# mhnazeri/PMoE

Measured on AMD Instinct MI355X. Metric: samples/sec fwd+bwd, 256x256 RGB 4-expert PMoE, higher is better.
Workload: dtype bf16; 1 GPU; 4-expert MoE (PMoE experts), 256x256x3 x4 frames, batch 64/GPU, fwd+moe_loss+bwd, dropout 0.3; global_batch=64, parallelism=dp1

## Files before the change

### include/pmoe_hip.h

```cpp
#ifndef PMOE_HIP_H
#define PMOE_HIP_H
#include <stdint.h>
#ifdef __cplusplus
extern "C" {
#endif

#define PMOE_DT_BF16 0
#define PMOE_DT_F32 1

#define PMOE_ERR_ARG (-1)
#define PMOE_ERR_UNSUPPORTED (-2)

#define PMOE_ACT_NONE 0
#define PMOE_ACT_RELU 1
#define PMOE_ACT_ELU 2
#define PMOE_ACT_TANH 3
#define PMOE_ACT_SIGMOID 4

#define PMOE_RES_NONE 0
#define PMOE_RES_ADD 1
#define PMOE_RES_DRELU 2
#define PMOE_RES_DELU 3
#define PMOE_RES_DTANH 4
#define PMOE_RES_DSIGMOID 5
// ... 4 lines not shown
int pmoe_version(void);
const char* pmoe_error_string(int code);
int pmoe_abi_sizeof(int which);

typedef struct pmoe_conv_desc {
    const void* in;
    const void* w;
    void* out;
    const void* res;
    const float* bias;
    float* stats;
    int32_t n, h, w_, cin;
    int32_t ho, wo, cout, coutp;
    int32_t in_ld, in_coff, out_ld, out_coff, res_ld, res_coff;
    int32_t ipe;
    int32_t in_shared;
    int32_t ks, stride, pad, dilate;
    int32_t act, res_mode;
    float drop_p;
    uint64_t seed;
    int32_t dtype;
    int32_t w_fp8;
    float in_scale;
    const float* out_scale;
    int32_t in_fp8;
    const float* bn_coef;
    int32_t bn_ipe;
    int32_t shuffle_c;
} pmoe_conv_desc;

int pmoe_conv2d_igemm(const pmoe_conv_desc* d, void* stream);
int pmoe_conv2d_stat_rows(const pmoe_conv_desc* d);
int pmoe_conv2d_plan(const pmoe_conv_desc* d);

typedef struct pmoe_wgrad_desc {
    const void* x;
    const void* dy;
    float* dw_ws;
    int32_t n, h, w_, cin, cinp;
    int32_t ho, wo, cout, coutp;
    int32_t x_ld, x_coff, dy_ld, dy_coff;
    int32_t ipe, x_shared;
    int32_t ks, stride, pad;
    int32_t dtype;
    int32_t per_image;
    float* part_ws;
    int64_t part_ws_floats;
    float* grads;
    int32_t cout_real, cin_real;
    int32_t defer_fold;
    int32_t bn_fused;
    const void* bn_z;
    const float* bn_coef;
    const float* bn_c1;
    const float* bn_c2;
    int32_t bn_z_ld;
} pmoe_wgrad_desc;
int pmoe_conv2d_wgrad(const pmoe_wgrad_desc* d, void* stream);
int pmoe_conv2d_wgrad_fold(const pmoe_wgrad_desc* d, void* stream);
int64_t pmoe_conv2d_wgrad_ws_floats(const pmoe_wgrad_desc* d);
int pmoe_conv2d_wgrad_plan(const pmoe_wgrad_desc* d);

int pmoe_mlp_wgrad(const void* x, const void* dy, float* grads, float* bias_grads, int32_t n, int32_t ipe, int32_t x_shared,
                   int32_t cin, int32_t cout, int32_t cin_real, int32_t cout_real, int32_t x_ld, int32_t x_coff,
                   int32_t dy_ld, int32_t dy_coff, int32_t dtype, void* stream);

// ... 241 lines not shown
```

### pmoe_amd/csrc/api.hip

```cpp
#include "common.h"
#include "kernels.h"

static ConvArgs to_args(const pmoe_conv_desc* d) {
    ConvArgs a;
    a.in = d->in; a.w = d->w; a.out = d->out; a.res = d->res; a.bias = d->bias; a.stats = d->stats;
    a.N = d->n; a.H = d->h; a.W = d->w_; a.Cin = d->cin;
    a.Ho = d->ho; a.Wo = d->wo; a.Cout = d->cout; a.CoutP = d->coutp;
    a.in_ld = d->in_ld; a.in_coff = d->in_coff; a.out_ld = d->out_ld; a.out_coff = d->out_coff;
    a.res_ld = d->res_ld; a.res_coff = d->res_coff;
    a.ipe = d->ipe; a.in_shared = d->in_shared;
    a.ks = d->ks; a.stride = d->stride; a.pad = d->pad; a.dilate = d->dilate;
    a.act = d->act; a.res_mode = (d->res || d->res_mode == PMOE_RES_INBN) ? d->res_mode : PMOE_RES_NONE;
    a.drop_p = d->drop_p; a.seed = d->seed;
    a.oscale = d->out_scale; a.in_scale = d->in_scale; a.w_fp8 = d->w_fp8; a.in_fp8 = d->in_fp8;
    a.bn = d->bn_coef; a.bn_ipe = d->bn_ipe > 0 ? d->bn_ipe : d->ipe;
    a.lTW = a.lTH = a.TN = a.n_groups = a.tiles_y = a.tiles_x = 0;
    a.kh = a.kw = d->ks; a.use_tapmap = 0; a.tapmap[0] = a.tapmap[1] = a.tapmap[2] = a.tapmap[3] = 0;
    a.out_step = 1; a.out_offy = a.out_offx = 0; a.OH = d->ho; a.OW = d->wo; a.prefetch = 0; a.stagger = 0;
    a.shuf_c = d->shuffle_c > 0 ? d->shuffle_c : 0;
    return a;
}

static int check_conv(const pmoe_conv_desc* d) {
    if (!d || !d->in || !d->w || !d->out) return PMOE_ERR_ARG;
    if (d->n <= 0 || d->h <= 0 || d->w_ <= 0 || d->ho <= 0 || d->wo <= 0 || d->ipe <= 0) return PMOE_ERR_ARG;
    const int ve = d->dtype == PMOE_DT_BF16 ? 8 : 4;
    if (d->in_fp8 && (!d->w_fp8 || d->dtype != PMOE_DT_BF16 || d->in_ld % 16 || d->in_coff % 16)) return PMOE_ERR_ARG;
    if (d->in_ld % ve || d->in_coff % ve || d->out_ld % ve || d->out_coff % ve) return PMOE_ERR_ARG;
    if (d->res && (d->res_ld % ve || d->res_coff % ve)) return PMOE_ERR_ARG;
    if (d->shuffle_c > 0 ? (d->cout != 4 * d->shuffle_c || d->shuffle_c % ve || d->out_coff + d->shuffle_c > d->out_ld || d->cout > d->coutp)
                         : (d->cout > d->coutp || d->out_coff + d->cout > d->out_ld)) return PMOE_ERR_ARG;
    if (d->in_coff + d->cin > d->in_ld) return PMOE_ERR_ARG;
    if (d->drop_p < 0.f || d->drop_p >= 1.f) return PMOE_ERR_ARG;
    if (d->res && d->res_mode == PMOE_RES_DBN &&
        (!d->bn_coef || !d->stats || d->dtype != PMOE_DT_BF16 || (d->bn_ipe > 0 && (d->bn_ipe % d->ipe || d->n % d->bn_ipe))))
        return PMOE_ERR_ARG;
    if (d->res_mode == PMOE_RES_INBN &&
        (d->res || !d->bn_coef || d->dtype != PMOE_DT_BF16 || (d->bias && d->ks != 1) || d->act != PMOE_ACT_NONE || d->drop_p != 0.f || d->in_shared ||
         d->w_fp8 || d->dilate || (d->bn_ipe > 0 && (d->bn_ipe % d->ipe || d->n % d->bn_ipe))))
        return PMOE_ERR_ARG;
    if (!d->dilate) {
        if (d->ho != (d->h + 2 * d->pad - d->ks) / d->stride + 1) return PMOE_ERR_ARG;
        if (d->wo != (d->w_ + 2 * d->pad - d->ks) / d->stride + 1) return PMOE_ERR_ARG;
    }
    return 0;
}

extern "C" {

int pmoe_version(void) { return PMOE_ABI_VERSION; }

int pmoe_abi_sizeof(int which) {
// ... 3 lines not shown
}

const char* pmoe_error_string(int code) {
    if (code == 0) return "ok";
    if (code == PMOE_ERR_ARG) return "pmoe: invalid argument (shape / alignment / pointer)";
    if (code == PMOE_ERR_UNSUPPORTED) return "pmoe: unsupported configuration (no tile fits LDS)";
    if (code > 0) return hipGetErrorString((hipError_t)code);
    return "pmoe: unknown error";
}

int pmoe_conv2d_igemm(const pmoe_conv_desc* d, void* stream) {
    int rc = check_conv(d);
    if (rc) return rc;
    return conv_igemm_launch(to_args(d), d->dtype, (hipStream_t)stream);
}

static ConvArgs to_plan_args(const pmoe_conv_desc* d) {
    ConvArgs a = to_args(d);
    if (a.in_ld <= 0) a.in_ld = a.in_coff + a.Cin;
    if (a.out_ld <= 0) a.out_ld = a.out_coff + a.Cout;
    return a;
}

int pmoe_conv2d_stat_rows(const pmoe_conv_desc* d) {
    if (!d || d->ipe <= 0) return PMOE_ERR_ARG;
    return conv_igemm_mblocks(to_plan_args(d), d->dtype);
}

int pmoe_conv2d_plan(const pmoe_conv_desc* d) {
    if (!d || d->ipe <= 0) return PMOE_ERR_ARG;
    return conv_igemm_plan(to_plan_args(d), d->dtype);
}

static int to_wgrad_args(const pmoe_wgrad_desc* d, WgradArgs& a) {
    if (!d || d->ipe <= 0) return PMOE_ERR_ARG;
    const int ve = d->dtype == PMOE_DT_BF16 ? 8 : 4;
    if (d->x_ld % ve || d->x_coff % ve || d->dy_ld % ve || d->dy_coff % ve) return PMOE_ERR_ARG;
    if (d->x_coff + d->cin > d->x_ld || d->dy_coff + d->cout > d->dy_ld) return PMOE_ERR_ARG;
    if (d->ho != (d->h + 2 * d->pad - d->ks) / d->stride + 1) return PMOE_ERR_ARG;
    if (d->wo != (d->w_ + 2 * d->pad - d->ks) / d->stride + 1) return PMOE_ERR_ARG;
    a.x = d->x; a.dy = d->dy; a.dw = d->dw_ws; a.part = d->part_ws; a.part_floats = d->part_ws_floats;
    a.N = d->n; a.H = d->h; a.W = d->w_; a.Cin = d->cin; a.CinP = d->cinp;
    a.Ho = d->ho; a.Wo = d->wo; a.Cout = d->cout; a.CoutP = d->coutp;
    a.x_ld = d->x_ld; a.x_coff = d->x_coff; a.dy_ld = d->dy_ld; a.dy_coff = d->dy_coff;
    a.ipe = d->ipe; a.x_shared = d->x_shared;
    a.ks = d->ks; a.stride = d->stride; a.pad = d->pad; a.per_image = d->per_image;
    a.grads = d->grads; a.cout_real = d->cout_real; a.cin_real = d->cin_real; a.defer_fold = d->defer_fold;
    if (a.grads && (a.per_image || a.cout_real <= 0 || a.cin_real <= 0 || a.cout_real > a.CoutP || a.cin_real > a.CinP)) return PMOE_ERR_ARG;
    a.lTW = a.lTH = a.TN = a.n_groups = a.tiles_y = a.tiles_x = a.mb_per_wg = 0;
    a.slice_fastest = 0;
    return 0;
}

static WgradBn to_wgrad_bn(const pmoe_wgrad_desc* d) { return {d->bn_fused, d->bn_z_ld, d->bn_z, d->bn_coef, d->bn_c1, d->bn_c2}; }

int pmoe_conv2d_wgrad(const pmoe_wgrad_desc* d, void* stream) {
    WgradArgs a;
    const int rc = to_wgrad_args(d, a);
    if (rc) return rc;
    if (!d->x || !d->dy || !d->dw_ws) return PMOE_ERR_ARG;
    return conv_wgrad_launch(a, d->dtype, to_wgrad_bn(d), (hipStream_t)stream);
}

int pmoe_conv2d_wgrad_fold(const pmoe_wgrad_desc* d, void* stream) {
    WgradArgs a;
    const int rc = to_wgrad_args(d, a);
// ... 19 lines not shown
```

### pmoe_amd/csrc/conv_igemm.hip

```cpp
#include "conv_common.h"
#include <stdlib.h>
#include <string.h>
#include "kernels.h"

template <int LOG_RB> __device__ __forceinline__ int swz(int x) { return swz_chunk<LOG_RB, 0>(x); }

template <typename T> struct Mma;
template <> struct Mma<bf16> {
    static __device__ __forceinline__ void run(const v4i& a, const v4i& b, f32x16& c) {
        c = __builtin_amdgcn_mfma_f32_32x32x16_bf16(__builtin_bit_cast(bf16x8, a), __builtin_bit_cast(bf16x8, b), c, 0, 0, 0);
    }
};
template <> struct Mma<float> {
    static __device__ __forceinline__ void run(const v4i& a, const v4i& b, f32x16& c) {
        const f32x4 fa = __builtin_bit_cast(f32x4, a), fb = __builtin_bit_cast(f32x4, b);
#pragma unroll
        for (int j = 0; j < 4; ++j) c = __builtin_amdgcn_mfma_f32_32x32x2f32(fa[j], fb[j], c, 0, 0, 0);
    }
};

template <> struct Mma<fp8> {
    static __device__ __forceinline__ void run(const v4i& a, const v4i& b, f32x16& c) {
        typedef long l2 __attribute__((ext_vector_type(2)));
        const l2 la = __builtin_bit_cast(l2, a), lb = __builtin_bit_cast(l2, b);
        c = __builtin_amdgcn_mfma_f32_32x32x16_fp8_fp8(la[0], lb[0], c, 0, 0, 0);
        c = __builtin_amdgcn_mfma_f32_32x32x16_fp8_fp8(la[1], lb[1], c, 0, 0, 0);
    }
};

#ifdef PMOE_STAMP
#define STAMP_INIT unsigned long long st_prev = __builtin_amdgcn_s_memtime(); unsigned st_acc[5] = {0, 0, 0, 0, 0};
#define LAP(i) { const unsigned long long st_t = __builtin_amdgcn_s_memtime(); st_acc[i] += (unsigned)(st_t - st_prev); st_prev = st_t; }
#else
#define STAMP_INIT
#define LAP(i)
// ... 315 lines not shown
        for (int i = 0; i < VE; ++i) {
#pragma unroll
            for (int off = CPO; off < 64; off <<= 1) {
                s1[i] += __shfl_xor(s1[i], off);
                s2[i] += __shfl_xor(s2[i], off);
            }
        }
        if (CPO >= 64 || lane < CPO) {
#pragma unroll
            for (int i = 0; i < VE; ++i) {
                red[(wave * 2 + 0) * BN + cc * VE + i] = s1[i];
                red[(wave * 2 + 1) * BN + cc * VE + i] = s2[i];
            }
        }
        __syncthreads();
        if (tid < 2 * BN) {
            const int which = tid / BN, c = tid % BN;
            float s = 0.f;
#pragma unroll
            for (int w = 0; w < WM * WN; ++w) s += red[(w * 2 + which) * BN + c];
            if (cout0 + c < a.CoutP) a.stats[((size_t)mb * 2 + which) * a.CoutP + cout0 + c] = s;
        }
    }
}

template <typename T, int LOG_RB, int WM, int WN, typename TL = T>
__global__ void __launch_bounds__(WM * WN * 64) conv_igemm_kernel(const ConvArgs a) {
    conv_igemm_body<T, LOG_RB, WM, WN, false, TL>(a);
}

template <typename T, int LOG_RB, typename TL = T>
__global__ void __launch_bounds__(512, 4) conv_igemm_lite_kernel(const ConvArgs a) {
    conv_igemm_body<T, LOG_RB, 4, 2, true, TL>(a);
}

template <typename T, int LOG_RB, typename TL = T>
static int launch_lite(const ConvArgs& a, int mblocks, size_t smem, hipStream_t st) {
    auto k = conv_igemm_lite_kernel<T, LOG_RB, TL>;
    HIP_RET((ensure_dyn_lds<conv_igemm_lite_kernel<T, LOG_RB, TL>>(160 * 1024)));
    dim3 grid(mblocks * (a.CoutP / 128), 1, 1), block(512, 1, 1);
    hipLaunchKernelGGL(k, grid, block, smem, st, a);
    return (int)hipGetLastError();
}

template <typename T, int LOG_RB, int WM, int WN, typename TL = T>
static int launch_cfg(const ConvArgs& a, int mblocks, size_t smem, hipStream_t st) {
    auto k = conv_igemm_kernel<T, LOG_RB, WM, WN, TL>;
    HIP_RET((ensure_dyn_lds<conv_igemm_kernel<T, LOG_RB, WM, WN, TL>>(160 * 1024)));
    dim3 grid(mblocks, a.CoutP / (WN * 64), 1), block(WM * WN * 64, 1, 1);
    hipLaunchKernelGGL(k, grid, block, smem, st, a);
    return (int)hipGetLastError();
}

static int env_switch(const char* name) { const char* ev = getenv(name); return ev ? atoi(ev) : 1; }

static int tile_plan(const ConvArgs& a, int tsz, int esz, ConvLaunch* l) {
    const bool F8 = esz != tsz;
    if (a.Cin <= 0 || a.CoutP % 64 || a.Cout % (16 / tsz) || a.Cin % (32 / esz)) return PMOE_ERR_ARG;
    if (F8 && a.Cin % 64) return PMOE_ERR_ARG;
    if ((a.ks != 1 && a.ks != 3) || (a.stride != 1 && a.stride != 2) || (a.dilate && a.stride != 1)) return PMOE_ERR_ARG;
    if (a.N % a.ipe) return PMOE_ERR_ARG;
    static const int cfg42 = env_switch("PMOE_CONV_CFG42"), lite_on = env_switch("PMOE_CONV_LITE"),
                     stg_on = env_switch("PMOE_CONV_STAGGER"), pf_on = env_switch("PMOE_CONV_PREFETCH");
    const int E = a.N / a.ipe;
    const bool wide = (a.CoutP % 128 == 0);
    const bool big = wide && cfg42 && tsz == 2 && (long long)a.ipe * a.Ho * a.Wo >= 4096;
// ... 41 lines not shown
static int tile_plan_dtype(const ConvArgs& a, int dtype, ConvLaunch* l) {
    return dtype == PMOE_DT_BF16 ? tile_plan(a, 2, 2, l) : dtype == PMOE_DT_F32 ? tile_plan(a, 4, 4, l) : PMOE_ERR_ARG;
}

template <typename T, typename TL = T> static int tile_launch(const ConvLaunch& l, hipStream_t st) {
    const ConvArgs& a = l.a;
    if (l.lite) return launch_lite<T, 7, TL>(a, l.mblocks, l.smem, st);
    switch (l.log_rb * 100 + l.wm * 10 + l.wn) {
    case 742: return launch_cfg<T, 7, 4, 2, TL>(a, l.mblocks, l.smem, st);
    case 642: return launch_cfg<T, 6, 4, 2, TL>(a, l.mblocks, l.smem, st);
    case 722: return launch_cfg<T, 7, 2, 2, TL>(a, l.mblocks, l.smem, st);
    case 741: return launch_cfg<T, 7, 4, 1, TL>(a, l.mblocks, l.smem, st);
    case 622: return launch_cfg<T, 6, 2, 2, TL>(a, l.mblocks, l.smem, st);
    case 641: return launch_cfg<T, 6, 4, 1, TL>(a, l.mblocks, l.smem, st);
    }
    if constexpr (sizeof(TL) == sizeof(T)) {
        switch (l.log_rb * 100 + l.wm * 10 + l.wn) {
        case 542: return launch_cfg<T, 5, 4, 2>(a, l.mblocks, l.smem, st);
        case 522: return launch_cfg<T, 5, 2, 2>(a, l.mblocks, l.smem, st);
        case 541: return launch_cfg<T, 5, 4, 1>(a, l.mblocks, l.smem, st);
        }
    }
    return PMOE_ERR_UNSUPPORTED;
}

static int launch_one(const ConvLaunch& l, int dtype, hipStream_t st) {
    switch (l.kind) {
    case CONV_SKINNY: return gemm_skinny_launch(l, st);
    case CONV_C16: return conv_c16_launch(l, st);
    case CONV_C1X1: return conv_c1x1_launch(l, st);
    case CONV_RES: return conv_res_launch(l, st);
    case CONV_DMA: case CONV_DMA_S2: case CONV_DMA_S2CLS: case CONV_DMA_F8: return conv_dma_launch(l, st);
    case CONV_TILE:
        if (l.a.w_fp8) return !l.a.oscale || !(l.a.in_scale > 0.f) ? PMOE_ERR_ARG : tile_launch<bf16, fp8>(l, st);
        return dtype == PMOE_DT_BF16 ? tile_launch<bf16>(l, st) : tile_launch<float>(l, st);
    }
    return PMOE_ERR_ARG;
}

static int select_stride2_dgrad(const ConvArgs& a, int dtype, ConvPlan* p) {
    p->n = 0;
    for (int py = 0; py < 2; ++py)
        for (int px = 0; px < 2; ++px) {
            ConvArgs c = a;
            c.dilate = 0; c.stride = 1; c.pad = 0;
            c.kh = 1 + py; c.kw = 1 + px;
            c.Ho = (a.Ho - py + 1) / 2; c.Wo = (a.Wo - px + 1) / 2;
            if (c.Ho <= 0 || c.Wo <= 0) continue;
            c.OH = a.Ho; c.OW = a.Wo; c.out_step = 2; c.out_offy = py; c.out_offx = px;
            c.use_tapmap = 1;
            for (int r = 0; r < c.kh; ++r)
                for (int q = 0; q < c.kw; ++q) {
                    const int fy = py ? (r == 0 ? 0 : 2) : 1, fx = px ? (q == 0 ? 0 : 2) : 1;
                    c.tapmap[r * c.kw + q] = fy * 3 + fx;
                }
            ConvLaunch* l = &p->l[p->n++];
            if (!conv_dma_s2cls_plan(c, dtype, l)) {
                const int rc = tile_plan_dtype(c, dtype, l);
                if (rc) return rc;
            }
        }
    if (!p->n) return PMOE_ERR_ARG;
    ConvLaunch t;
    const int esz = dtype == PMOE_DT_BF16 ? 2 : 4, rc = tile_plan(a, esz, esz, &t);
    p->mblocks = rc ? rc : t.mblocks;
    return 4000 + p->l[p->n - 1].code;
}

int conv_select(const ConvArgs& a, int dtype, ConvPlan* p) {
    memset(p, 0, sizeof(*p));
    p->n = 1;
    ConvLaunch* l = p->l;
    int code = 0;
    const bool bn_mode = a.res_mode == PMOE_RES_INBN || a.res_mode == PMOE_RES_DBN;
    if (a.in_fp8 && !a.w_fp8) {
        code = PMOE_ERR_UNSUPPORTED;
    } else if (a.shuf_c) {
        code = conv_c1x1_plan(a, dtype, l) ? 0 : PMOE_ERR_UNSUPPORTED;
    } else if (a.w_fp8) {
        if (dtype != PMOE_DT_BF16 || a.dilate) code = PMOE_ERR_ARG;
        else if (a.in_fp8) code = conv_dma_f8_plan(a, dtype, l) ? 0 : PMOE_ERR_UNSUPPORTED;
        else if (bn_mode) code = PMOE_ERR_UNSUPPORTED;
        else code = tile_plan(a, 2, 1, l);
    } else if (a.res_mode == PMOE_RES_INBN) {
        if (!(!a.bias && conv_res_plan(a, dtype, l) && l->res_pipe) && !conv_c1x1_plan(a, dtype, l))
            code = PMOE_ERR_UNSUPPORTED;
    } else if (a.res_mode == PMOE_RES_DBN) {
        if (!(conv_res_plan(a, dtype, l) && l->res_dma) && (gemm_skinny_plan(a, dtype, l) || !conv_dma_plan(a, dtype, l)))
            code = PMOE_ERR_UNSUPPORTED;
    } else if (a.dilate && a.ks == 3 && a.pad == 1 && a.kh == 3) {
        const int code = select_stride2_dgrad(a, dtype, p);
        if (code < 0) p->n = 0;
        return p->code = code;
    } else if (a.dilate && a.ks == 1 && a.pad == 0 && a.res_mode == PMOE_RES_ADD && a.res == a.out && a.res_ld == a.out_ld &&
               a.res_coff == a.out_coff && !a.bias && a.act == PMOE_ACT_NONE && a.drop_p == 0.f) {
        ConvArgs c = a;
        c.dilate = 0; c.stride = 1; c.pad = 0; c.kh = c.kw = 1;
        c.Ho = (a.Ho + 1) / 2; c.Wo = (a.Wo + 1) / 2;
        c.OH = a.Ho; c.OW = a.Wo; c.out_step = 2; c.out_offy = c.out_offx = 0;
        code = tile_plan_dtype(c, dtype, l);
    } else if (!gemm_skinny_plan(a, dtype, l) && !conv_c16_plan(a, dtype, l) && !conv_c1x1_plan(a, dtype, l) &&
               !conv_res_plan(a, dtype, l) && !conv_dma_plan(a, dtype, l) && !conv_dma_s2_plan(a, dtype, l)) {
        code = tile_plan_dtype(a, dtype, l);
    }
    if (code < 0) { p->n = 0; return p->code = code; }
    p->mblocks = l->mblocks;
    return p->code = l->code;
}

int conv_igemm_launch(const ConvArgs& a, int dtype, hipStream_t st) {
    ConvPlan p;
    const int code = conv_select(a, dtype, &p);
    if (code < 0) return code;
    for (int i = 0; i < p.n; ++i) {
        const int rc = launch_one(p.l[i], dtype, st);
        if (rc) return rc;
    }
    return 0;
}

int conv_igemm_plan(const ConvArgs& a, int dtype) {
    ConvPlan p;
    return conv_select(a, dtype, &p);
}

int conv_igemm_mblocks(const ConvArgs& a, int dtype) {
    static float rows_only;
    ConvArgs s = a;
    if (!s.stats) s.stats = &rows_only;
    ConvPlan p;
    const int code = conv_select(s, dtype, &p);
    return code < 0 ? code : p.mblocks;
}
```

### pmoe_amd/csrc/kernels.h

```cpp
#pragma once
#include <hip/hip_runtime.h>
#include <stdint.h>
#include "../../include/pmoe_hip.h"

struct ConvArgs {
    const void* in;
    const void* w;
    void* out;
    const void* res;
    const float* bias;
    float* stats;
    const float* oscale;
    float in_scale;
    int w_fp8;
    int in_fp8;
    int N, H, W, Cin;
    int Ho, Wo, Cout, CoutP;
    int in_ld, in_coff, out_ld, out_coff, res_ld, res_coff;
    int ipe;
    int in_shared;
    int ks, stride, pad, dilate;
    int act, res_mode;
    float drop_p;
    unsigned long long seed;
    int lTW, lTH, TN, n_groups, tiles_y, tiles_x;
    int kh, kw, use_tapmap, tapmap[4];
    int out_step, out_offy, out_offx, OH, OW;
    const float* bn;
    int bn_ipe;
    int stagger;
    int prefetch;
    int shuf_c;
};

struct WgradArgs {
    const void* x;
    const void* dy;
    float* dw;
    float* part;
    long long part_floats;
    int N, H, W, Cin, CinP;
    int Ho, Wo, Cout, CoutP;
    int x_ld, x_coff, dy_ld, dy_coff;
    int ipe, x_shared;
    int ks, stride, pad;
    int per_image;
    float* grads;
    int cout_real, cin_real;
    int defer_fold;
    int lTW, lTH, TN, n_groups, tiles_y, tiles_x, mb_per_wg;
    int slice_fastest;
};

inline bool magic_div_exact(int n, int PW, int PH, int* mpw, int* mph) {
    *mpw = 65536 / PW + 1; *mph = 65536 / PH + 1;
    for (int pp = 0; pp < n; ++pp)
        if (((pp * *mpw) >> 16) != pp / PW || (((pp / PW) * *mph) >> 16) != (pp / PW) / PH) return false;
    return true;
}

struct ResPlan {
    int lTW, lTH, TN, n_groups, tiles_y, tiles_x, tiles_per_expert, wgs_per_expert, log_rb;
    size_t smem;
};

// ... 9 lines not shown
    int mf16, stream, producer, narrow;
    ResPlan res;
    int res_dma, res_pipe, rz_late;
    int wpe, tpe, tiles_x, slabs, mt;
    int log_rb, wm, wn, lite;
    int nw;
};

struct ConvPlan {
    int code;
    int mblocks;
    int n;
    ConvLaunch l[4];
};
int conv_select(const ConvArgs& a, int dtype, ConvPlan* p);

bool gemm_skinny_plan(const ConvArgs& a, int dtype, ConvLaunch* l);
int gemm_skinny_launch(const ConvLaunch& l, hipStream_t st);
bool conv_c16_plan(const ConvArgs& a, int dtype, ConvLaunch* l);
int conv_c16_launch(const ConvLaunch& l, hipStream_t st);
bool conv_c1x1_plan(const ConvArgs& a, int dtype, ConvLaunch* l);
int conv_c1x1_launch(const ConvLaunch& l, hipStream_t st);
bool conv_res_plan(const ConvArgs& a, int dtype, ConvLaunch* l);
int conv_res_launch(const ConvLaunch& l, hipStream_t st);
bool conv_dma_plan(const ConvArgs& a, int dtype, ConvLaunch* l);
bool conv_dma_f8_plan(const ConvArgs& a, int dtype, ConvLaunch* l);
bool conv_dma_s2_plan(const ConvArgs& a, int dtype, ConvLaunch* l);
bool conv_dma_s2cls_plan(const ConvArgs& a, int dtype, ConvLaunch* l);
int conv_dma_launch(const ConvLaunch& l, hipStream_t st);

int conv_igemm_launch(const ConvArgs& a, int dtype, hipStream_t st);
int conv_igemm_mblocks(const ConvArgs& a, int dtype);
int conv_igemm_plan(const ConvArgs& a, int dtype);

enum WgradKind { WGRAD_TILE = 1, WGRAD_DMA, WGRAD_DMA2, WGRAD_BNBWD };

struct WgradBn {
    int fused, z_ld;
    const void* z;
    const float *coef, *c1, *c2;
};

struct WgradPlan {
    int kind;
    int code;
    WgradArgs a;
    int esz, maxv;
    int pin, wci, pairs, req;
    int ahead;
    dim3 grid, block;
    size_t smem;
    int mpw, mph;
    int E, taps, nsplit;
    long long ws_floats;
};
int wgrad_select(const WgradArgs& a, int dtype, const WgradBn& bn, WgradPlan* p);

int conv_wgrad_launch(const WgradArgs& a, int dtype, const WgradBn& bn, hipStream_t st);
int conv_wgrad_fold(const WgradArgs& a, int dtype, const WgradBn& bn, hipStream_t st);
long long conv_wgrad_ws_floats(const WgradArgs& a, int dtype, const WgradBn& bn);
int conv_wgrad_plan(const WgradArgs& a, int dtype, const WgradBn& bn);
```

### pmoe_amd/hip.py

```python
import ctypes as C
import os
from pathlib import Path

import torch

_LIB_PATH = Path(os.environ.get("PMOE_HIP_LIB") or Path(__file__).resolve().parent / "libpmoe_hip.so")
_lib = None

ABI_VERSION = 401
DT_BF16, DT_F32 = 0, 1
ACT_NONE, ACT_RELU, ACT_ELU, ACT_TANH, ACT_SIGMOID = 0, 1, 2, 3, 4
RES_NONE, RES_ADD, RES_DRELU, RES_DELU, RES_DTANH, RES_DSIGMOID, RES_DBN, RES_INBN = 0, 1, 2, 3, 4, 5, 6, 7
ERR_ARG, ERR_UNSUPPORTED = -1, -2
RES_OF_ACT = {ACT_RELU: RES_DRELU, ACT_ELU: RES_DELU, ACT_TANH: RES_DTANH, ACT_SIGMOID: RES_DSIGMOID}
ACT_BY_NAME = {"relu": ACT_RELU, "elu": ACT_ELU, "tanh": ACT_TANH, "sigmoid": ACT_SIGMOID}

_TORCH_DT = {torch.bfloat16: DT_BF16, torch.float32: DT_F32}


class HipUnavailable(RuntimeError):
    pass


class ConvDesc(C.Structure):
# ... 7 lines not shown
        ("ipe", C.c_int32), ("in_shared", C.c_int32),
        ("ks", C.c_int32), ("stride", C.c_int32), ("pad", C.c_int32), ("dilate", C.c_int32),
        ("act", C.c_int32), ("res_mode", C.c_int32),
        ("drop_p", C.c_float), ("seed", C.c_uint64), ("dtype", C.c_int32),
        ("w_fp8", C.c_int32), ("in_scale", C.c_float), ("out_scale", C.c_void_p),
        ("in_fp8", C.c_int32), ("bn_coef", C.c_void_p), ("bn_ipe", C.c_int32), ("shuffle_c", C.c_int32),
    ]


class WgradDesc(C.Structure):
    _fields_ = [
        ("x", C.c_void_p), ("dy", C.c_void_p), ("dw_ws", C.c_void_p),
        ("n", C.c_int32), ("h", C.c_int32), ("w_", C.c_int32), ("cin", C.c_int32), ("cinp", C.c_int32),
        ("ho", C.c_int32), ("wo", C.c_int32), ("cout", C.c_int32), ("coutp", C.c_int32),
        ("x_ld", C.c_int32), ("x_coff", C.c_int32), ("dy_ld", C.c_int32), ("dy_coff", C.c_int32),
        ("ipe", C.c_int32), ("x_shared", C.c_int32),
        ("ks", C.c_int32), ("stride", C.c_int32), ("pad", C.c_int32), ("dtype", C.c_int32),
        ("per_image", C.c_int32),
        ("part_ws", C.c_void_p), ("part_ws_floats", C.c_int64),
        ("grads", C.c_void_p), ("cout_real", C.c_int32), ("cin_real", C.c_int32), ("defer_fold", C.c_int32),
        ("bn_fused", C.c_int32), ("bn_z", C.c_void_p), ("bn_coef", C.c_void_p), ("bn_c1", C.c_void_p), ("bn_c2", C.c_void_p),
        ("bn_z_ld", C.c_int32),
    ]


_P, _I, _L, _F = C.c_void_p, C.c_int32, C.c_int64, C.c_float
SIGNATURES = {
    "pmoe_version": [],
    "pmoe_error_string": [C.c_int],
    "pmoe_abi_sizeof": [C.c_int],
    "pmoe_conv2d_igemm": [C.POINTER(ConvDesc), _P],
    "pmoe_conv2d_stat_rows": [C.POINTER(ConvDesc)],
    "pmoe_conv2d_plan": [C.POINTER(ConvDesc)],
    "pmoe_conv2d_wgrad": [C.POINTER(WgradDesc), _P],
    "pmoe_conv2d_wgrad_fold": [C.POINTER(WgradDesc), _P],
    "pmoe_conv2d_wgrad_ws_floats": [C.POINTER(WgradDesc)],
    "pmoe_conv2d_wgrad_plan": [C.POINTER(WgradDesc)],
    "pmoe_mlp_wgrad": [_P, _P, _P, _P, _I, _I, _I, _I, _I, _I, _I, _I, _I, _I, _I, _I, _P],
    "pmoe_bn_apply_pool2": [_P, _P, _P, _P, _P, _P, _I, _I, _I, _I, _I, _I, _I, _I, _I, _P],
    "pmoe_pack_conv_weights": [_P, _P, _P, _I, _I, _I, _I, _I, _I, _I, _I, _I, _P],
    "pmoe_pack_conv_weights_fp8": [_P, _P, _P, _P, _P, _F, _I, _I, _I, _I, _I, _I, _I, _I, _P],
    "pmoe_pack_conv_weights_scaled": [_P, _P, _P, _P, _P, _P, _I, _I, _I, _I, _I, _I, _I, _P],
    "pmoe_pack_conv_weights_gated": [_P, _P, _I, _P, _P, _I, _I, _I, _I, _I, _I, _I, _I, _I, _I, _P],
    "pmoe_unpack_conv_wgrad": [_P, _P, _I, _I, _I, _I, _I, _I, _P],
    "pmoe_pack_bias": [_P, _P, _I, _I, _I, _P],
    "pmoe_act_fwd": [_P, _P, _L, _I, _F, C.c_uint64, _I, _P],
    "pmoe_act_bwd": [_P, _P, _P, _L, _I, _F, _I, _P],
    "pmoe_colstats": [_P, _L, _I, _I, _I, _I, _P, _I, _P, _I, _P],
    "pmoe_reduce_partials": [_P, _P, _I, _I, _I, _I, _P],
    "pmoe_bn_finalize": [_P, _I, _L, _P, _P, _P, _P, _F, _F, _I, _P, _P, _P, _P, _I, _I, _P, _P],
    "pmoe_bn_apply": [_P, _P, _P, _P, _P, _P, _L, _I, _I, _I, _I, _I, _I, _P, _F, _P],
    "pmoe_bn_bwd_reduce": [_P, _P, _P, _P, _P, _P, _P, _L, _I, _I, _I, _P, _I, _P, _I, _P],
    "pmoe_bn_bwd_finalize": [_P, _I, _L, _P, _P, _P, _P, _I, _I, _P],
    "pmoe_bn_bwd_apply": [_P, _P, _P, _P, _P, _P, _P, _P, _P, _P, _P, _L, _I, _I, _I, _I, _P],
    "pmoe_stem_tail_stats": [_P, _P, _P, _P, _P, _I, _P, _P, _I, _I, _I, _I, _I, _I, _P],
    "pmoe_stem_tail_pooled": [_P, _P, _P, C.POINTER(C.c_void_p), _P, _I, _I, _L, _I, _I, _P],
    "pmoe_stem_tail_combine": [_P, _I, _P, _I, C.POINTER(C.c_void_p), _L, _P, _P, _I, _I, _P],
    "pmoe_stem_tail_pool": [_P, _P, _P, _P, _P, _P, _P, _P, _P, _I, _I, _I, _I, _I, _I, _P],
    "pmoe_stem_tail_bwd": [_I, _P, _P, _P, _P, C.POINTER(C.c_void_p), _P, _I, _I, _I, _I, _I, _I, _I, _P],
    "pmoe_maxpool3s2_fwd": [_P, _P, _P, _I, _I, _I, _I, _I, _P],
    "pmoe_maxpool3s2_bwd": [_P, _P, _P, _I, _I, _I, _I, _I, _P],
    "pmoe_gap_partial": [_P, _P, _P, _I, _L, _I, _I, _I, _I, _P],
    "pmoe_bn_apply_gap": [_P, _P, _P, _P, _P, _P, _I, _I, _I, _L, _I, _I, _I, _P],
    "pmoe_gap_finish": [_P, _P, _I, _I, _I, _L, _I, _I, _I, _P],
    "pmoe_gap_bwd": [_P, _P, _I, _L, _I, _I, _I, _I, _P],
    "pmoe_eca_gate": [_P, _I, _L, _P, _I, _P, _P, _I, _I, _I, _I, _I, _P],
# ... 20 lines not shown
    "pmoe_pixel_unshuffle2": [_P, _I, _I, _P, _I, _I, _I, _I, _I, _I, _P],
    "pmoe_add_window": [_P, _I, _I, _P, _I, _I, _L, _I, _I, _P],
    "pmoe_cat_windows": [C.POINTER(C.c_void_p), _I, _I, _I, _I, _P, _I, _I, _L, _I, _P],
    "pmoe_nhwc_to_nchw": [_P, _I, _I, _P, _I, _L, _I, _I, _P],
    "pmoe_seg_loss_rows": [_I, _I, _I],
    "pmoe_seg_loss_cp": [_I],
    "pmoe_seg_loss_fwd": [_P, _P, _I, _I, _I, _I, _I, _I, _F, _F, _F, _F, _P, _P, _P, _P, _P, _P],
    "pmoe_seg_loss_bwd": [_P, _P, _P, _P, _P, _P, _I, _I, _I, _I, _I, _I, _P],
    "pmoe_dice_score": [_P, _P, _I, _I, _L, _F, _P, _P, _P],
    "pmoe_dropout2d_table": [_P, _I, _I, _F, C.c_uint64, _P],
    "pmoe_channel_scale": [_P, _I, _I, _P, _I, _L, _I, _I, _P],
    "pmoe_resample_u8_horizontal": [_P, _P, _I, _I, _I, _I, _I, _I, _I, _P, _P, _I, _P],
    "pmoe_resample_u8_vertical_to_f32": [_P, _P, _I, _I, _I, _I, _I, _P, _P, _I, _P],
    "pmoe_resample_u8_vertical_to_i64": [_P, _P, _I, _I, _I, _I, _I, _P, _P, _I, _P],
    "pmoe_resample_u8_vertical_to_u8": [_P, _P, _I, _I, _I, _I, _I, _P, _P, _I, _P],
    "pmoe_augment_point_to_u8": [_P, _P, _P, _I, _I, _I, _I, _P],
    "pmoe_augment_point_to_f32": [_P, _P, _P, _I, _I, _I, _I, _P],
    "pmoe_augment_blur_h": [_P, _P, _P, _I, _I, _I, _P],
    "pmoe_augment_blur_v": [_P, _P, _P, _I, _I, _I, _P],
    "pmoe_mt_grad_norm": [_P, _P, _P, _I, _F, _P, _P, _I, _P],
    "pmoe_mt_adam": [_P, _P, _P, _I, _F, _F, _F, _F, _F, _I, _F, _F, _P, _P],
    "pmoe_mt_adam_packs": [_P, _P, _P, _P, _P, _I, _F, _F, _F, _F, _F, _I, _F, _F, _P, _P],
    "pmoe_mt_swa_update": [_P, _P, _P, _I, _L, _P],
}
_RESTYPES = {"pmoe_error_string": C.c_char_p, "pmoe_conv2d_wgrad_ws_floats": C.c_int64}


def lib_path():
    return _LIB_PATH


_recorder = None
_NOT_LAUNCHES = frozenset(("pmoe_error_string", "pmoe_abi_sizeof", "pmoe_conv2d_plan", "pmoe_conv2d_stat_rows",
                           "pmoe_conv2d_wgrad_plan", "pmoe_conv2d_wgrad_ws_floats"))


class LaunchRecorder:

    def __init__(self):
        self.calls = []
        self.stream = None

    def __enter__(self):
        global _recorder
        if _recorder is not None:
            raise RuntimeError("a LaunchRecorder is already active")
        self.stream = torch.cuda.current_stream().cuda_stream
        _recorder = self
        return self

    def __exit__(self, *exc):
        global _recorder
        _recorder = None
        return False

    def replay(self):
        if torch.cuda.current_stream().cuda_stream != self.stream:
            raise RuntimeError("LaunchRecorder.replay: the plan was recorded on another stream")
        for fn, args in self.calls:
            rc = fn(*args)
            if rc:
                check(rc, fn.__name__)


class _RecordingLib:
    def __init__(self, lib, rec):
        self._lib, self._rec = lib, rec
# ... 70 lines not shown
```

### pmoe_amd/ops.py

```python
import ctypes as C

import torch

from . import hip
from .hip import ConvDesc, WgradDesc, check, dt, load, ptr, stream_ptr


def _round_up(v, m):
    return (v + m - 1) // m * m


def conv_out_size(h, ks, stride, pad):
    return (h + 2 * pad - ks) // stride + 1


def _nhwc(t, name):
    if t.dim() != 4:
        raise ValueError(f"{name}: expected NHWC [N,H,W,C], got shape {tuple(t.shape)}")
    return t.shape


def _conv_desc(n, h, w_, ho, wo, cin, cout, coutp, ipe, ks, stride, pad, dtype, *, dilate=False, in_shared=False, in_ld=0,
               in_coff=0, out_ld=0, out_coff=0, res_mode=hip.RES_NONE, res_ld=0, res_coff=0, act=hip.ACT_NONE, drop_p=0.0, seed=0,
               w_fp8=False, in_fp8=False, in_scale=1.0, bn_ipe=0, shuffle2_c=0):
# ... 12 lines not shown
    if res_mode in (hip.RES_DBN, hip.RES_INBN):
        d.bn_ipe = int(bn_ipe or ipe)
    return d


def _stand_in(t, name=None, dtype=None):
    return None if t is None else C.c_void_p(id(t))


def _planning_desc(n, h, w_, ho, wo, cin, cout, coutp, ipe, ks, stride, pad, dtype, bias=False, stats=False, **kw):
    d = _conv_desc(n, h, w_, ho, wo, cin, cout, coutp, ipe, ks, stride, pad, hip._TORCH_DT[dtype], **kw)
    d.in_, d.w, d.out = 1, 2, 3
    if d.res_mode not in (hip.RES_NONE, hip.RES_INBN):
        d.res = 4
    if d.res_mode in (hip.RES_DBN, hip.RES_INBN):
        d.bn_coef = 5
    if d.w_fp8:
        d.out_scale = 6
    d.bias, d.stats = (7 if bias else None), (8 if stats else None)
    return d


class ConvLaunch:
    __slots__ = ("d", "out", "stats")

    def __init__(self, d, out, stats):
        self.d, self.out, self.stats = d, out, stats

    def plan(self):
        return load().pmoe_conv2d_plan(C.byref(self.d))

    def served(self):
        return self.plan() >= 0

    def stat_rows(self):
        return _stat_rows(self.d)

    def launch(self):
        return _conv2d_launch(self)


def _stat_rows(d):
    rows = load().pmoe_conv2d_stat_rows(C.byref(d))
    if rows < 0:
        check(rows, "pmoe_conv2d_stat_rows")
    return rows


def _conv2d_launch(p):
    d = p.d
    if p.out is None:
        raise ValueError("conv2d: a launch prepared from shapes only can be asked, not run")
    if p.stats is not None:
        rows = p.stat_rows()
        if p.stats is True:
            p.stats = torch.empty(rows, 2, d.coutp, dtype=torch.float32, device=p.out.device)
        elif p.stats.dim() != 3 or p.stats.shape[0] != rows or p.stats.shape[1] != 2 or p.stats.shape[2] != d.coutp:
            raise ValueError(f"conv2d: stats must be [{rows}, 2, {d.coutp}] for this launch, got {tuple(p.stats.shape)}")
        d.stats = ptr(p.stats, "stats", torch.float32)
    elif d.res_mode == hip.RES_DBN:
        raise ValueError("conv2d: RES_DBN writes the BatchNorm-backward reductions to `stats`")
    if _prof is not None:
        _launch_info["kernel"] = p.plan()
    check(load().pmoe_conv2d_igemm(C.byref(d), stream_ptr()), "pmoe_conv2d_igemm")
    return p.out

# ... 23 lines not shown
                   res_mode=res_mode if (res is not None or res_mode == hip.RES_INBN) else hip.RES_NONE,
                   res_ld=res.shape[-1] if res is not None else 0, res_coff=res_coff, act=act, drop_p=drop_p, seed=seed,
                   w_fp8=w_fp8, in_fp8=in_fp8, in_scale=in_scale, bn_ipe=bn_ipe, shuffle2_c=shuffle2_c)
    d.in_, d.w, d.out, d.res, d.bias, d.stats = in_, w, o, res_p, bias_p, stats_p
    if w_fp8:
        d.out_scale = at(out_scale, "out_scale", torch.float32)
    if d.res_mode in (hip.RES_DBN, hip.RES_INBN):
        inbn = d.res_mode == hip.RES_INBN
        want = (4, n // (bn_ipe or ipe), cin if inbn else cout)
        if (inbn and res is not None) or bn_coef is None or bn_coef.dtype != torch.float32 or tuple(bn_coef.shape) != want:
            raise ValueError(f"conv2d: RES_{'INBN takes no `res` and' if inbn else 'DBN'} needs bn_coef {list(want)} f32")
        d.bn_coef = at(bn_coef, "bn_coef", torch.float32)
    if in_shared and nin != ipe:
        raise ValueError("conv2d: shared input must hold exactly ipe images")
    if not in_shared and nin != n:
        raise ValueError("conv2d: input/output image counts differ")
    if w_packed.numel() < (n // ipe) * coutp * ks * ks * cin:
        raise ValueError("conv2d: packed weight tensor too small")
    return ConvLaunch(d, None if shapes_only else out, stats)


def conv2d(x, w_packed, out, *, plan_only=False, **kw):
    if kw.get("stats") is True:
        raise ValueError("conv2d: stats=True (the launch allocates the buffer) is conv2d_prepare's: conv2d returns only `out`")
    p = conv2d_prepare(x, w_packed, out, **kw)
    return p.plan() if plan_only else p.launch()


def conv2d_plan(n, h, w_, ho, wo, cin, cout, coutp, ipe, ks, stride, pad, dtype, *, bias=False, stats=False, **kw):
    return load().pmoe_conv2d_plan(C.byref(_planning_desc(n, h, w_, ho, wo, cin, cout, coutp, ipe, ks, stride, pad, dtype,
                                                          bias=bias, stats=stats, **kw)))


def conv2d_stat_rows(n, h, w_, ho, wo, cin, cout, coutp, ipe, ks, stride, pad, dtype, w_fp8=False, in_ld=0, out_ld=0,
                     in_shared=False, in_fp8=False):
    return _stat_rows(_planning_desc(n, h, w_, ho, wo, cin, cout, coutp, ipe, ks, stride, pad, dtype, w_fp8=w_fp8, in_fp8=in_fp8,
                                     in_ld=in_ld, out_ld=out_ld, in_shared=in_shared))


_wgrad_scratch = {}


def _wgrad_part_ws(device, floats):
    key = (device, torch.cuda.current_stream(device).cuda_stream)
    buf = _wgrad_scratch.get(key)
    if buf is None or buf.numel() < floats:
        buf = _wgrad_scratch[key] = torch.empty(max(floats, 1 << 22), dtype=torch.float32, device=device)
    return buf


def _wgrad_desc(n, h, w_, ho, wo, cin, cout, cinp, coutp, ipe, ks, stride, pad, dtype, *, x_ld=0, dy_ld=0, x_coff=0, dy_coff=0,
                x_shared=False, per_image=False, bn_z_ld=None):
    d = WgradDesc()
    d.n, d.h, d.w_, d.cin, d.cinp = n, h, w_, cin, cinp
    d.ho, d.wo, d.cout, d.coutp = ho, wo, cout, coutp
    d.x_ld, d.x_coff, d.dy_ld, d.dy_coff = x_ld or x_coff + cin, x_coff, dy_ld or dy_coff + cout, dy_coff
    d.ipe, d.x_shared = ipe, int(x_shared)
    d.ks, d.stride, d.pad, d.dtype = ks, stride, pad, dtype
    d.per_image = int(per_image)
    if bn_z_ld is not None:
        d.bn_fused, d.bn_z_ld = 1, bn_z_ld or d.dy_ld
    return d


def _wgrad_ws(d):
    need = load().pmoe_conv2d_wgrad_ws_floats(C.byref(d))
# ... 600 lines not shown
```

Baseline: 1901 samples/s.

## Fuse four stride-2 dgrad phase launches into one s2-walk kernel

Adds a new kernel that computes all four output parity phases of a stride-2 3x3 data-gradient convolution in a single launch. It loads each input halo patch once per channel chunk and walks the taps of the phases in pairs, with double-buffered weight slices. Before, four separate tile kernels each reloaded the patch. The fused path is enabled by default (env PMOE_S2_FUSE) when all four sub-plans are bf16 tile 4x1 configs, and it adds a launch-count query API. The cost is extra registers from two accumulator sets and serialized epilogues.

```diff
diff --git a/include/pmoe_hip.h b/include/pmoe_hip.h
--- a/include/pmoe_hip.h
+++ b/include/pmoe_hip.h
@@ -60,6 +60,7 @@
 int pmoe_conv2d_igemm(const pmoe_conv_desc* d, void* stream);
 int pmoe_conv2d_stat_rows(const pmoe_conv_desc* d);
 int pmoe_conv2d_plan(const pmoe_conv_desc* d);
+int pmoe_conv2d_launches(const pmoe_conv_desc* d);
 
 typedef struct pmoe_wgrad_desc {
     const void* x;
diff --git a/pmoe_amd/csrc/api.hip b/pmoe_amd/csrc/api.hip
--- a/pmoe_amd/csrc/api.hip
+++ b/pmoe_amd/csrc/api.hip
@@ -18,6 +18,7 @@
     a.kh = a.kw = d->ks; a.use_tapmap = 0; a.tapmap[0] = a.tapmap[1] = a.tapmap[2] = a.tapmap[3] = 0;
     a.out_step = 1; a.out_offy = a.out_offx = 0; a.OH = d->ho; a.OW = d->wo; a.prefetch = 0; a.stagger = 0;
     a.shuf_c = d->shuffle_c > 0 ? d->shuffle_c : 0;
+    a.s2_walk = 0;
     return a;
 }
 
@@ -87,6 +88,11 @@
     return conv_igemm_plan(to_plan_args(d), d->dtype);
 }
 
+int pmoe_conv2d_launches(const pmoe_conv_desc* d) {
+    if (!d || d->ipe <= 0) return PMOE_ERR_ARG;
+    return conv_igemm_launches(to_plan_args(d), d->dtype);
+}
+
 static int to_wgrad_args(const pmoe_wgrad_desc* d, WgradArgs& a) {
     if (!d || d->ipe <= 0) return PMOE_ERR_ARG;
     const int ve = d->dtype == PMOE_DT_BF16 ? 8 : 4;
diff --git a/pmoe_amd/csrc/conv_igemm.hip b/pmoe_amd/csrc/conv_igemm.hip
--- a/pmoe_amd/csrc/conv_igemm.hip
+++ b/pmoe_amd/csrc/conv_igemm.hip
@@ -1,6 +1,7 @@
 #include "conv_common.h"
 #include <stdlib.h>
 #include <string.h>
+#include <type_traits>
 #include "kernels.h"
 
 template <int LOG_RB> __device__ __forceinline__ int swz(int x) { return swz_chunk<LOG_RB, 0>(x); }
@@ -382,6 +383,247 @@
 template <typename T, int LOG_RB, typename TL = T>
 __global__ void __launch_bounds__(512, 4) conv_igemm_lite_kernel(const ConvArgs a) {
     conv_igemm_body<T, LOG_RB, 4, 2, true, TL>(a);
+}
+
+template <typename T, int LOG_RB, int WM, int WN>
+__global__ void __launch_bounds__(WM * WN * 64, 2) conv_igemm_s2walk_kernel(const ConvArgs a) {
+    constexpr int RB = 1 << LOG_RB, CPR = RB / 16, LOG_CPR = LOG_RB - 4;
+    constexpr int NTHR = WM * WN * 64;
+    constexpr int BM = WM * 64, BN = WN * 64;
+    constexpr int VE = 16 / (int)sizeof(T);
+    constexpr int CK = RB / (int)sizeof(T);
+    constexpr int KSUB = RB / 32;
+    constexpr int TAPS = 9;
+    extern __shared__ __attribute__((aligned(16))) char smem[];
+
+    const int tid = threadIdx.x, lane = tid & 63, wave = tid >> 6;
+    const int l31 = lane & 31, h = lane >> 5;
+    const int wm = wave / WN, wn = wave % WN;
+
+    const unsigned mb = xcd_remap(blockIdx.x, gridDim.x);
+    const int nb = (int)blockIdx.y;
+    int t = (int)mb;
+    const int tx = t % a.tiles_x; t /= a.tiles_x;
+    const int ty = t % a.tiles_y; t /= a.tiles_y;
+    const int ng = t % a.n_groups;
+    const int e = t / a.n_groups;
+    const int lTW = a.lTW, lTH = a.lTH;
+    const int TW = 1 << lTW, TH = 1 << lTH;
+    const int PW = TW + 1, PH = TH + 1;
+    const int NPIX = a.TN * PH * PW;
+    const int n0 = e * a.ipe + ng * a.TN, n_end = (e + 1) * a.ipe;
+    const int oy0 = ty * TH, ox0 = tx * TW;
+    const int cout0 = nb * BN;
+
+    const int PB = (NPIX * RB + 255) & ~255;
+    char* patch = smem;
+    char* wbuf = smem + PB;
+
+    int ppb[2];
+#pragma unroll
+    for (int mt = 0; mt < 2; ++mt) {
+        const int p = wm * 64 + mt * 32 + l31;
+        const int mx = p & (TW - 1), my = (p >> lTW) & (TH - 1), pn = p >> (lTW + lTH);
+        ppb[mt] = (pn * PH + my) * PW + mx;
+    }
+
+    const T* wbase = (const T*)a.w + ((size_t)e * a.CoutP + cout0) * TAPS * a.Cin;
+    constexpr int WV = (BN * CPR + NTHR - 1) / NTHR;
+    v4i wreg[WV];
+    auto w_issue = [&](int c0, int tap) {
+#pragma unroll
+        for (int i = 0; i < WV; ++i) {
+            const int v = tid + i * NTHR;
+            if (v < BN * CPR) {
+                const int n = v >> LOG_CPR, j = v & (CPR - 1);
+                wreg[i] = ldg16(wbase + ((size_t)n * TAPS + tap) * a.Cin + c0 + j * VE);
+            }
+        }
+    };
+    auto w_commit = [&](int buf) {
+#pragma unroll
+        for (int i = 0; i < WV; ++i) {
+            const int v = tid + i * NTHR;
+            if (v < BN * CPR) {
+                const int n = v >> LOG_CPR, j = v & (CPR - 1);
+                *reinterpret_cast<v4i*>(wbuf + buf * (BN * RB) + n * RB + ((j ^ swz<LOG_RB>(n)) << 4)) = wreg[i];
+            }
+        }
+    };
+
+    PatchGeom geo;
+    geo.n0 = n0; geo.n_end = n_end; geo.e_first_img = e * a.ipe;
+    geo.Y0 = oy0; geo.X0 = ox0; geo.PH = PH; geo.PW = PW; geo.NPIX = NPIX;
+    geo.H = a.H; geo.W = a.W; geo.ld = a.in_ld; geo.coff = a.in_coff; geo.cmax = a.Cin;
+    geo.dilate = 0; geo.shared = a.in_shared; geo.step = 1;
+    const T* in = (const T*)a.in;
+    auto load_patch = [&](int c0) { load_halo_patch<T, LOG_RB, NTHR, 0>(patch, in, geo, c0, tid); };
+
+    int cur = 0;
+    auto tap_step = [&](f32x16 (&acc)[2][2], int r, int q, bool has_next, int nc0, int ntap) {
+        if (has_next) w_issue(nc0, ntap);
+        const char* wb = wbuf + cur * (BN * RB);
+        const int tapoff = r * PW + q;
+        int pp[2], fp[2];
+#pragma unroll
+        for (int mt = 0; mt < 2; ++mt) {
+            pp[mt] = ppb[mt] + tapoff;
+            fp[mt] = swz<LOG_RB>(pp[mt]);
+        }
+#pragma unroll
+        for (int ks = 0; ks < KSUB; ++ks) {
+            v4i af[2], bfr[2];
+#pragma unroll
+            for (int nt = 0; nt < 2; ++nt) {
+                const int row = wn * 64 + nt * 32 + l31;
+                af[nt] = *reinterpret_cast<const v4i*>(wb + row * RB + (((ks * 2 + h) ^ swz<LOG_RB>(row)) << 4));
+            }
+#pragma unroll
+            for (int mt = 0; mt < 2; ++mt)
+                bfr[mt] = *reinterpret_cast<const v4i*>(patch + pp[mt] * RB + (((ks * 2 + h) ^ fp[mt]) << 4));
+#pragma unroll
+            for (int nt = 0; nt < 2; ++nt)
+#pragma unroll
+                for (int mt = 0; mt < 2; ++mt) Mma<T>::run(af[nt], bfr[mt], acc[nt][mt]);
+        }
+        if (has_next) w_commit(cur ^ 1);
+        __syncthreads();
+        cur ^= 1;
+    };
+
+    constexpr int UPR = BN / 4;
+    float* stg = reinterpret_cast<float*>(smem);
+    constexpr int CPO = BN / VE;
+    constexpr int PROWS = NTHR / CPO;
+    const int cc = tid % CPO, pr = tid / CPO;
+    const int cout = cout0 + cc * VE;
+    const bool cvalid = cout < a.Cout;
+    const float keep_scale = a.drop_p > 0.f ? 1.f / (1.f - a.drop_p) : 1.f;
+    T* out = (T*)a.out;
+    const T* res = (const T*)a.res;
+    auto epilogue = [&](const f32x16 (&acc)[2][2], int cy, int cx) {
+        const int Hc = (a.OH - cy + 1) >> 1, Wc = (a.OW - cx + 1) >> 1;
+        float bias[VE];
+#pragma unroll
+        for (int i = 0; i < VE; ++i) bias[i] = (a.bias && cvalid) ? a.bias[(size_t)e * a.CoutP + cout + i] : 0.f;
+#pragma unroll
+        for (int nt = 0; nt < 2; ++nt)
+#pragma unroll
+            for (int mt = 0; mt < 2; ++mt) {
+                const int p = wm * 64 + mt * 32 + l31;
+#pragma unroll
+                for (int g = 0; g < 4; ++g) {
+                    const int u = wn * 16 + nt * 8 + 2 * g + h;
+                    f32x4 v;
+#pragma unroll
+                    for (int i = 0; i < 4; ++i) v[i] = acc[nt][mt][4 * g + i];
+                    *reinterpret_cast<f32x4*>(stg + p * BN + ((u ^ (p & (UPR - 1))) << 2)) = v;
+                }
+            }
+        __syncthreads();
+        for (int p = pr; p < BM; p += PROWS) {
+            const int mx = p & (TW - 1), my = (p >> lTW) & (TH - 1), pn = p >> (lTW + lTH);
+            const int n = n0 + pn, oy = oy0 + my, ox = ox0 + mx;
+            if (!(cvalid && n < n_end && oy < Hc && ox < Wc)) continue;
+            float v[VE];
+#pragma unroll
+            for (int k = 0; k < VE / 4; ++k) {
+                const int u = cc * (VE / 4) + k;
+                const f32x4 tt = *reinterpret_cast<const f32x4*>(stg + p * BN + ((u ^ (p & (UPR - 1))) << 2));
+#pragma unroll
+                for (int i = 0; i < 4; ++i) v[4 * k + i] = tt[i];
+            }
+            const size_t opix = ((size_t)n * a.OH + oy * 2 + cy) * a.OW + ox * 2 + cx;
+#pragma unroll
+            for (int i = 0; i < VE; ++i) v[i] += bias[i];
+            if (a.res_mode) {
+                float rv[VE];
+                unpack16<T>(ldg16(res + opix * a.res_ld + a.res_coff + cout), rv);
+                if (a.res_mode == PMOE_RES_ADD) {
+#pragma unroll
+                    for (int i = 0; i < VE; ++i) v[i] += rv[i];
+                } else if (a.res_mode == PMOE_RES_DRELU) {
+#pragma unroll
+                    for (int i = 0; i < VE; ++i) v[i] = rv[i] > 0.f ? v[i] * keep_scale : 0.f;
+                } else if (a.res_mode >= PMOE_RES_DELU) {
+#pragma unroll
+                    for (int i = 0; i < VE; ++i) {
+                        const float y = rv[i] * (1.f / keep_scale);
+                        const float d = act_deriv_from_output(a.res_mode, y);
+                        v[i] = (a.drop_p > 0.f && rv[i] == 0.f) ? 0.f : v[i] * d * keep_scale;
+                    }
+                }
+            }
+            if (a.act == PMOE_ACT_RELU) {
+#pragma unroll
+                for (int i = 0; i < VE; ++i) v[i] = fmaxf(v[i], 0.f);
+            } else if (a.act != PMOE_ACT_NONE) {
+#pragma unroll
+                for (int i = 0; i < VE; ++i) v[i] = act_apply(a.act, v[i]);
+            }
+            if (a.drop_p > 0.f && a.res_mode < PMOE_RES_DRELU) {
+                const unsigned long long base = (unsigned long long)opix * (unsigned)a.Cout + cout;
+#pragma unroll
+                for (int i = 0; i < VE; ++i)
+                    v[i] = hash_uniform(a.seed, base + i) >= a.drop_p ? v[i] * keep_scale : 0.f;
+            }
+            stg16(out + opix * a.out_ld + a.out_coff + cout, pack16<T>(v));
+        }
+    };
+
+    const int nchunks = a.Cin / CK;
+    auto run_pair = [&](auto pair_c) {
+        constexpr int PAIR = decltype(pair_c)::value;
+        f32x16 acc[2][2][2];
+#pragma unroll
+        for (int s = 0; s < 2; ++s)
+#pragma unroll
+            for (int i = 0; i < 2; ++i)
+#pragma unroll
+                for (int j = 0; j < 2; ++j)
+#pragma unroll
+                    for (int k = 0; k < 16; ++k) acc[s][i][j][k] = 0.f;
+        for (int ch = 0; ch < nchunks; ++ch) {
+            const int c0 = ch * CK;
+            const bool more = ch + 1 < nchunks;
+            load_patch(c0);
+            __syncthreads();
+            if constexpr (PAIR == 0) {
+                tap_step(acc[0], 0, 0, true, c0, 2);
+                tap_step(acc[0], 0, 1, true, c0, 6);
+                tap_step(acc[0], 1, 0, true, c0, 8);
+                tap_step(acc[0], 1, 1, true, c0, 4);
+                tap_step(acc[1], 0, 0, more, c0 + CK, 0);
+            } else {
+                tap_step(acc[0], 0, 0, true, c0, 5);
+                tap_step(acc[0], 0, 1, true, c0, 1);
+                tap_step(acc[1], 0, 0, true, c0, 7);
+                tap_step(acc[1], 1, 0, more, c0 + CK, 3);
+            }
+        }
+        if constexpr (PAIR == 0) w_issue(0, 3);
+        epilogue(acc[0], PAIR == 0 ? 1 : 0, 1);
+        __syncthreads();
+        epilogue(acc[1], PAIR == 0 ? 0 : 1, 0);
+        if constexpr (PAIR == 0) {
+            __syncthreads();
+            cur = 0;
+            w_commit(0);
+        }
+    };
+    w_issue(0, 0);
+    w_commit(0);
+    run_pair(std::integral_constant<int, 0>{});
+    run_pair(std::integral_constant<int, 1>{});
+}
+
+template <typename T, int LOG_RB, int WM, int WN>
+static int launch_s2walk(const ConvArgs& a, int mblocks, size_t smem, hipStream_t st) {
+    auto k = conv_igemm_s2walk_kernel<T, LOG_RB, WM, WN>;
+    HIP_RET((ensure_dyn_lds<conv_igemm_s2walk_kernel<T, LOG_RB, WM, WN>>(160 * 1024)));
+    dim3 grid(mblocks, a.CoutP / (WN * 64), 1), block(WM * WN * 64, 1, 1);
+    hipLaunchKernelGGL(k, grid, block, smem, st, a);
+    return (int)hipGetLastError();
 }
 
 template <typename T, int LOG_RB, typename TL = T>
@@ -489,10 +731,29 @@
     case CONV_RES: return conv_res_launch(l, st);
     case CONV_DMA: case CONV_DMA_S2: case CONV_DMA_S2CLS: case CONV_DMA_F8: return conv_dma_launch(l, st);
     case CONV_TILE:
+        if (l.a.s2_walk) return launch_s2walk<bf16, 7, 4, 1>(l.a, l.mblocks, l.smem, st);
         if (l.a.w_fp8) return !l.a.oscale || !(l.a.in_scale > 0.f) ? PMOE_ERR_ARG : tile_launch<bf16, fp8>(l, st);
         return dtype == PMOE_DT_BF16 ? tile_launch<bf16>(l, st) : tile_launch<float>(l, st);
     }
     return PMOE_ERR_ARG;
+}
+
+static bool s2_walk_plan(const ConvArgs& a, int dtype, const ConvPlan& four, ConvLaunch* l) {
+    if (dtype != PMOE_DT_BF16 || four.n != 4 || a.stats || a.w_fp8 || a.in_fp8 || a.shuf_c) return false;
+    if (a.res_mode == PMOE_RES_INBN || a.res_mode == PMOE_RES_DBN) return false;
+    for (int i = 0; i < 4; ++i) {
+        const ConvLaunch& c = four.l[i];
+        if (c.kind != CONV_TILE || c.lite || c.log_rb != 7 || c.wm != 4 || c.wn != 1) return false;
+    }
+    ConvArgs c = a;
+    c.dilate = 0; c.stride = 1; c.pad = 0;
+    c.kh = c.kw = 2;
+    c.Ho = (a.Ho + 1) / 2; c.Wo = (a.Wo + 1) / 2;
+    c.OH = a.Ho; c.OW = a.Wo; c.out_step = 2; c.out_offy = c.out_offx = 0;
+    c.use_tapmap = 0;
+    c.s2_walk = 1;
+    if (tile_plan(c, 2, 2, l)) return false;
+    return !l->lite && l->log_rb == 7 && l->wm == 4 && l->wn == 1 && !l->a.prefetch && l->smem >= (size_t)256 * 64 * 4;
 }
 
 static int select_stride2_dgrad(const ConvArgs& a, int dtype, ConvPlan* p) {
@@ -521,7 +782,13 @@
     ConvLaunch t;
     const int esz = dtype == PMOE_DT_BF16 ? 2 : 4, rc = tile_plan(a, esz, esz, &t);
     p->mblocks = rc ? rc : t.mblocks;
-    return 4000 + p->l[p->n - 1].code;
+    const int code = 4000 + p->l[p->n - 1].code;
+    const char* ev = getenv("PMOE_S2_FUSE");
+    if ((!ev || atoi(ev)) && s2_walk_plan(a, dtype, *p, &t) && 4000 + t.code == code) {
+        p->l[0] = t;
+        p->n = 1;
+    }
+    return code;
 }
 
 int conv_select(const ConvArgs& a, int dtype, ConvPlan* p) {
@@ -581,6 +848,12 @@
     return conv_select(a, dtype, &p);
 }
 
+int conv_igemm_launches(const ConvArgs& a, int dtype) {
+    ConvPlan p;
+    const int code = conv_select(a, dtype, &p);
+    return code < 0 ? code : p.n;
+}
+
 int conv_igemm_mblocks(const ConvArgs& a, int dtype) {
     static float rows_only;
     ConvArgs s = a;
diff --git a/pmoe_amd/csrc/kernels.h b/pmoe_amd/csrc/kernels.h
--- a/pmoe_amd/csrc/kernels.h
+++ b/pmoe_amd/csrc/kernels.h
@@ -31,6 +31,7 @@
     int stagger;
     int prefetch;
     int shuf_c;
+    int s2_walk;
 };
 
 struct WgradArgs {
@@ -106,6 +107,7 @@
 int conv_igemm_launch(const ConvArgs& a, int dtype, hipStream_t st);
 int conv_igemm_mblocks(const ConvArgs& a, int dtype);
 int conv_igemm_plan(const ConvArgs& a, int dtype);
+int conv_igemm_launches(const ConvArgs& a, int dtype);
 
 enum WgradKind { WGRAD_TILE = 1, WGRAD_DMA, WGRAD_DMA2, WGRAD_BNBWD };
 
diff --git a/pmoe_amd/hip.py b/pmoe_amd/hip.py
--- a/pmoe_amd/hip.py
+++ b/pmoe_amd/hip.py
@@ -63,6 +63,7 @@
     "pmoe_conv2d_igemm": [C.POINTER(ConvDesc), _P],
     "pmoe_conv2d_stat_rows": [C.POINTER(ConvDesc)],
     "pmoe_conv2d_plan": [C.POINTER(ConvDesc)],
+    "pmoe_conv2d_launches": [C.POINTER(ConvDesc)],
     "pmoe_conv2d_wgrad": [C.POINTER(WgradDesc), _P],
     "pmoe_conv2d_wgrad_fold": [C.POINTER(WgradDesc), _P],
     "pmoe_conv2d_wgrad_ws_floats": [C.POINTER(WgradDesc)],
@@ -149,7 +150,7 @@
 
 _recorder = None
 _NOT_LAUNCHES = frozenset(("pmoe_error_string", "pmoe_abi_sizeof", "pmoe_conv2d_plan", "pmoe_conv2d_stat_rows",
-                           "pmoe_conv2d_wgrad_plan", "pmoe_conv2d_wgrad_ws_floats"))
+                           "pmoe_conv2d_launches", "pmoe_conv2d_wgrad_plan", "pmoe_conv2d_wgrad_ws_floats"))
 
 
 class LaunchRecorder:
diff --git a/pmoe_amd/ops.py b/pmoe_amd/ops.py
--- a/pmoe_amd/ops.py
+++ b/pmoe_amd/ops.py
@@ -68,6 +68,9 @@
 
     def served(self):
         return self.plan() >= 0
+
+    def launches(self):
+        return load().pmoe_conv2d_launches(C.byref(self.d))
 
     def stat_rows(self):
         return _stat_rows(self.d)
@@ -157,6 +160,11 @@
                                                           bias=bias, stats=stats, **kw)))
 
 
+def conv2d_launches(n, h, w_, ho, wo, cin, cout, coutp, ipe, ks, stride, pad, dtype, *, bias=False, stats=False, **kw):
+    return load().pmoe_conv2d_launches(C.byref(_planning_desc(n, h, w_, ho, wo, cin, cout, coutp, ipe, ks, stride, pad, dtype,
+                                                              bias=bias, stats=stats, **kw)))
+
+
 def conv2d_stat_rows(n, h, w_, ho, wo, cin, cout, coutp, ipe, ks, stride, pad, dtype, w_fp8=False, in_ld=0, out_ld=0,
                      in_shared=False, in_fp8=False):
     return _stat_rows(_planning_desc(n, h, w_, ho, wo, cin, cout, coutp, ipe, ks, stride, pad, dtype, w_fp8=w_fp8, in_fp8=in_fp8,
```

Measured after the change: 1890 samples/s. About the same (-0.6%).
